# MisEty/RTG-SLAM

Hardware: AMD Instinct MI355X
Metric: hot_path_units_per_sec (higher is better)
Workload: dtype f32; 1 GPU; `value` counts UNITS, not SLAM frames (the SLAM frame rate by the reference's definition is `slam_frames_per_sec`, from the `slam_sequence` leg of --full).  One UNIT per step = 1 ICP track (3 levels x 5 GN iters, 1200x680, on a second HIP stream) + 1 map-optimisation iteration (raster fwd + masked L1 colour / gated depth loss + attach regulariser + raster bwd + fused Adam) over 1200000 random Gaus; gaussians=1200000, mode=single, parallelism=1 GPU

## Files before the change

include/rtgs_debug.h:

```cpp
#ifndef RTGS_DEBUG_H
#define RTGS_DEBUG_H
#include "rtgs_raster.h"
#ifdef __cplusplus
extern "C" {
#endif

void rtgs_raster_set_counters(void* counters);
void rtgs_raster_set_counters_ctx(rtgs_ctx* ctx, void* counters);

void rtgs_raster_set_profiling(int enable);
void rtgs_raster_set_profiling_ctx(rtgs_ctx* ctx, int enable);

void rtgs_raster_set_near_slice(int mode, int budget_per_tile);
void rtgs_raster_set_near_slice_ctx(rtgs_ctx* ctx, int mode, int budget_per_tile);

void rtgs_raster_force_sort_path(int enable);
void rtgs_raster_force_sort_path_ctx(rtgs_ctx* ctx, int enable);
int rtgs_raster_last_timings(float* ms12_host);
int rtgs_raster_last_timings_ctx(rtgs_ctx* ctx, float* ms12_host);

void rtgs_raster_set_bwd_walk_ctx(rtgs_ctx* ctx, int mode);
void rtgs_raster_set_onepass_ctx(rtgs_ctx* ctx, int on);
void rtgs_raster_set_fused_sort_ctx(rtgs_ctx* ctx, int on);
int rtgs_raster_fused_sort_stats_ctx(rtgs_ctx* ctx, int64_t* out18);
void rtgs_raster_set_tile_gather_ctx(rtgs_ctx* ctx, int mode);
int rtgs_raster_tile_gather_stats_ctx(rtgs_ctx* ctx, int64_t* out6);
void rtgs_raster_set_bwd_debug(int bits);
void rtgs_raster_set_bwd_stamps(void* dev);
void rtgs_raster_set_fwd_stamps(void* dev);
#define RTGS_ICP_STAMP_LAUNCHES 16
#define RTGS_ICP_STAMP_WGS 256
void rtgs_icp_set_stamps(void* dev);
void rtgs_tsdf_set_dense(int on);

#ifdef __cplusplus
}
#endif
#endif
```

rtg_slam_amd/csrc/map_fused.hip:

```cpp
#include "../../include/rtgs_raster.h"
#include "raster_common.h"
#include "raster_chain.h"
#include "adam_common.h"
#include "activate_common.h"

#include <math.h>

namespace rtgs {

struct FusedArgs {
  RasterParams p;
  const float *opac, *scales, *rots, *normal_w;
  const uint8_t* clamped;
  const BwdInfo* info;
  const uint32_t* gbase;
  uint32_t* slot_count;
  uint8_t* touched;
  SplatGrad* records;
  float *xyz, *shs, *raw8;
  float *m_xyz, *v_xyz, *m_shs, *v_shs, *m_raw8, *v_raw8;
  const float *lr_xyz, *lr_shs, *lr_raw8;
  uint8_t *ever_xyz, *ever_shs, *ever_raw8;
  float beta1, beta2, eps, bc1, bc2_sqrt;
  const float* init_xyz;
  const float4* init_raw8;
  const float* attach_info;
  float* confidence;
  float *act_opacity, *act_scales, *act_normal;
  float4* act_rots;
  uint32_t* live_counts;
  uint8_t* marks;
  int t0, rows;
};

constexpr int BIG_RUN = 8;

__device__ __forceinline__ bool attach_sel(const float4 init_lo) {
  return 1.f / (1.f + __expf(-init_lo.x)) < 0.9f;
}

template <int FCHUNK, int RPW = 64>
__global__ void __launch_bounds__(256) map_fused_tail_kernel(FusedArgs a) {
  __shared__ uint32_t s_list[FCHUNK];
  __shared__ uint32_t s_n;
  __shared__ float s_big[4][64][16];
  __shared__ float s_sh[4][64][20];
  __shared__ int s_rows[4][64];
  if (spec_failed(a.p.spec_fail)) return;
  const int tid = threadIdx.x, lane = tid & 63, wv = tid >> 6;
  const bool use_slots = a.info->use_slots != 0;
  const float* __restrict__ slots = reinterpret_cast<const float*>(a.info->slot_grads);
  uint32_t n_grad = 0, n_step = 0;
  for (int c0 = blockIdx.x * FCHUNK; c0 < a.rows; c0 += gridDim.x * FCHUNK) {
    __syncthreads();
    if (tid == 0) s_n = 0;
    __syncthreads();
    constexpr int PASSES = FCHUNK >= 256 ? FCHUNK / 256 : 1;
    uint32_t flags = 0;
#pragma unroll
    for (int k = 0; k < PASSES; ++k) {
      const int rl = min(c0 + k * 256 + tid, a.rows - 1);
      const uint32_t f = (uint32_t)a.touched[a.t0 + rl] | (uint32_t)a.ever_raw8[rl] | (uint32_t)a.ever_xyz[rl] | (uint32_t)a.ever_shs[rl];
      flags |= (f != 0u ? 1u : 0u) << k;
    }
#pragma unroll
    for (int k = 0; k < PASSES; ++k) {
      const int rl = c0 + k * 256 + tid;
      const bool work = rl < a.rows && k * 256 + tid < FCHUNK && ((flags >> k) & 1u) != 0u;
      const unsigned long long m = __builtin_amdgcn_ballot_w64(work);
      if (m == 0ull) continue;
      uint32_t base = 0;
      if (lane == 0) base = atomicAdd(&s_n, (uint32_t)__popcll(m));
      base = (uint32_t)__builtin_amdgcn_readfirstlane((int)base);
      if (work) s_list[base + (uint32_t)__popcll(m & ((1ull << lane) - 1ull))] = (uint32_t)rl;
    }
    __syncthreads();
    const int nlive = (int)s_n;
    for (int q0 = wv * RPW; q0 < nlive; q0 += 4 * RPW) {
      const int q = q0 + lane;
      const bool have = lane < RPW && q < nlive;
      const int rl = have ? (int)s_list[q] : 0;
      const int r = a.t0 + rl;
      bool rgrad = have && a.touched[r] != 0;
      SplatGrad g{};
      uint32_t cnt = 0, b0 = 0;
      if (rgrad && use_slots) { cnt = a.slot_count[r]; b0 = a.gbase[r]; }
      if (use_slots) {
        unsigned long long bigm = __builtin_amdgcn_ballot_w64(rgrad && cnt > (uint32_t)BIG_RUN);
        while (bigm != 0ull) {
          const int src = __builtin_ctzll(bigm);
          bigm &= bigm - 1ull;
          const uint32_t n = (uint32_t)__builtin_amdgcn_readlane((int)cnt, src);
          const size_t base = (size_t)(uint32_t)__builtin_amdgcn_readlane((int)b0, src);
          if (n <= 48u) {
            const int grp = lane >> 4, c = lane & 15;
            float m0 = 0.f, m1 = 0.f;
            uint32_t s = grp;
            for (; s + 4 < n; s += 8) { m0 += slots[(base + s) * 16 + c]; m1 += slots[(base + s + 4) * 16 + c]; }
            if (s < n) m0 += slots[(base + s) * 16 + c];
            float acc = m0 + m1;
            acc += __shfl_xor(acc, 16);
            acc += __shfl_xor(acc, 32);
            if (lane < 16) s_big[wv][src][c] = acc;
          } else {
            const float4* __restrict__ s4 = reinterpret_cast<const float4*>(slots);
            const uint32_t sub = (uint32_t)lane & 3u, sg = (uint32_t)lane >> 2;
            float4 a0 = make_float4(0.f, 0.f, 0.f, 0.f), a1 = a0, a2 = a0, a3 = a0;
            uint32_t s = sg;
            for (; s + 48 < n; s += 64) {
              const float4 t0 = s4[(base + s) * 4 + sub], t1 = s4[(base + s + 16) * 4 + sub];
              const float4 t2 = s4[(base + s + 32) * 4 + sub], t3 = s4[(base + s + 48) * 4 + sub];
              a0.x += t0.x; a0.y += t0.y; a0.z += t0.z; a0.w += t0.w; a1.x += t1.x; a1.y += t1.y; a1.z += t1.z; a1.w += t1.w;
              a2.x += t2.x; a2.y += t2.y; a2.z += t2.z; a2.w += t2.w; a3.x += t3.x; a3.y += t3.y; a3.z += t3.z; a3.w += t3.w;
            }
            for (; s < n; s += 16) {
              const float4 t0 = s4[(base + s) * 4 + sub];
              a0.x += t0.x; a0.y += t0.y; a0.z += t0.z; a0.w += t0.w;
            }
            float4 acc = make_float4((a0.x + a1.x) + (a2.x + a3.x), (a0.y + a1.y) + (a2.y + a3.y), (a0.z + a1.z) + (a2.z + a3.z),
                                     (a0.w + a1.w) + (a2.w + a3.w));
#pragma unroll
            for (int off = 4; off < 64; off <<= 1) {
              acc.x += __shfl_xor(acc.x, off); acc.y += __shfl_xor(acc.y, off);
              acc.z += __shfl_xor(acc.z, off); acc.w += __shfl_xor(acc.w, off);
            }
            if (lane < 4) { s_big[wv][src][4 * sub] = acc.x; s_big[wv][src][4 * sub + 1] = acc.y; s_big[wv][src][4 * sub + 2] = acc.z; s_big[wv][src][4 * sub + 3] = acc.w; }
          }
        }
        __builtin_amdgcn_wave_barrier();
        if (rgrad) {
          float t[16];
          if (cnt > (uint32_t)BIG_RUN) {
#pragma unroll
            for (int c = 0; c < 16; ++c) t[c] = s_big[wv][lane][c];
          } else {
#pragma unroll
            for (int c = 0; c < 16; ++c) t[c] = 0.f;
            const float4* s4 = reinterpret_cast<const float4*>(slots) + (size_t)b0 * 4;
            for (uint32_t s = 0; s < cnt; ++s) {
              const float4 x0 = s4[s * 4], x1 = s4[s * 4 + 1], x2 = s4[s * 4 + 2], x3 = s4[s * 4 + 3];
              t[0] += x0.x; t[1] += x0.y; t[2] += x0.z; t[3] += x0.w; t[4] += x1.x; t[5] += x1.y; t[6] += x1.z; t[7] += x1.w;
              t[8] += x2.x; t[9] += x2.y; t[10] += x2.z; t[11] += x2.w; t[12] += x3.x;
            }
          }
          g.du = t[0]; g.dv = t[1]; g.dca = t[2]; g.dcb = t[3]; g.dcc = t[4]; g.dop = t[5]; g.dr = t[6]; g.dg = t[7];
          g.db = t[8]; g.dnx = t[9]; g.dny = t[10]; g.dnz = t[11]; g.dpd = t[12];
          a.slot_count[r] = 0u;
        }
      } else if (rgrad) {
        g = a.records[r];
        float4* z = reinterpret_cast<float4*>(a.records + r);
        z[0] = z[1] = z[2] = z[3] = make_float4(0.f, 0.f, 0.f, 0.f);
      }
      if (rgrad) {
        a.touched[r] = 0;
        rgrad = (g.du != 0.f) | (g.dv != 0.f) | (g.dca != 0.f) | (g.dcb != 0.f) | (g.dcc != 0.f) | (g.dop != 0.f) |
                (g.dr != 0.f) | (g.dg != 0.f) | (g.db != 0.f) | (g.dnx != 0.f) | (g.dny != 0.f) | (g.dnz != 0.f) | (g.dpd != 0.f);
      }
      bool need_sh = false;
      if (have) {
        const uint8_t e_raw8 = a.ever_raw8[rl], e_xyz = a.ever_xyz[rl], e_shs = a.ever_shs[rl];
        ChainOut o{};
        if (rgrad) chain_rule(a.p, r, a.xyz, a.shs, a.scales, a.rots, a.normal_w, a.clamped, g, o, nullptr);
        const float4* raw8_4 = reinterpret_cast<const float4*>(a.raw8);
        float4 at_lo = make_float4(0.f, 0.f, 0.f, 0.f), at_hi = at_lo;
        float at[3] = {0.f, 0.f, 0.f};
        bool sel = false;
        if (a.init_raw8 && (rgrad || e_raw8 != 0 || e_xyz != 0)) {
          const float4 i_lo = a.init_raw8[2 * (size_t)rl];
          sel = attach_sel(i_lo);
          if (sel) {
            const float4 i_hi = a.init_raw8[2 * (size_t)rl + 1], c_lo = raw8_4[2 * (size_t)r], c_hi = raw8_4[2 * (size_t)r + 1];
            const float n = fmaxf(a.attach_info[0], 1.f);
            const float k3 = 2000.f / (n * 3.f), k4 = 2000.f / (n * 4.f);
            at_lo = make_float4(0.f, k3 * (c_lo.y - i_lo.y), k3 * (c_lo.z - i_lo.z), k3 * (c_lo.w - i_lo.w));
            at_hi = make_float4(k4 * (c_hi.x - i_hi.x), k4 * (c_hi.y - i_hi.y), k4 * (c_hi.z - i_hi.z), k4 * (c_hi.w - i_hi.w));
#pragma unroll
            for (int c = 0; c < 3; ++c) at[c] = k3 * (a.xyz[(size_t)r * 3 + c] - a.init_xyz[(size_t)rl * 3 + c]);
          }
        }
        const bool grad = rgrad || sel;
        if (a.marks && (grad || e_raw8 != 0 || e_xyz != 0)) a.marks[r] = 1;
        if (grad || e_raw8 != 0) {
          float4 lo = make_float4(0.f, 0.f, 0.f, 0.f), hi = lo;
          if (rgrad)
            activate8_bwd_row(raw8_4[2 * (size_t)r], raw8_4[2 * (size_t)r + 1], o.dop, o.ds[0], o.ds[1], o.ds[2], o.dq, o.dn[0],
                              o.dn[1], o.dn[2], lo, hi);
          lo.y += at_lo.y; lo.z += at_lo.z; lo.w += at_lo.w;
          hi.x += at_hi.x; hi.y += at_hi.y; hi.z += at_hi.z; hi.w += at_hi.w;
          if (e_raw8 == 0) a.ever_raw8[rl] = 1;
          float4* p4 = reinterpret_cast<float4*>(a.raw8) + 2 * (size_t)r;
          float4* m4 = reinterpret_cast<float4*>(a.m_raw8) + 2 * (size_t)rl;
          float4* v4 = reinterpret_cast<float4*>(a.v_raw8) + 2 * (size_t)rl;
          const float gg[8] = {lo.x, lo.y, lo.z, lo.w, hi.x, hi.y, hi.z, hi.w};
          float4 pp[2] = {p4[0], p4[1]}, mm[2] = {m4[0], m4[1]}, vv[2] = {v4[0], v4[1]};
          float* pf = reinterpret_cast<float*>(pp); float* mf = reinterpret_cast<float*>(mm); float* vf = reinterpret_cast<float*>(vv);
#pragma unroll
          for (int c = 0; c < 8; ++c) pf[c] = adam1(pf[c], gg[c], mf[c], vf[c], a.lr_raw8[c], a.beta1, a.beta2, a.eps, a.bc1, a.bc2_sqrt);
          p4[0] = pp[0]; p4[1] = pp[1]; m4[0] = mm[0]; m4[1] = mm[1]; v4[0] = vv[0]; v4[1] = vv[1];
          if (a.act_opacity) activate8_row_store(pp[0], pp[1], r, a.act_opacity, a.act_scales, a.act_rots, a.act_normal);
        }
        if (grad || e_xyz != 0) {
          if (e_xyz == 0) a.ever_xyz[rl] = 1;
#pragma unroll
          for (int c = 0; c < 3; ++c) {
            const size_t op = (size_t)r * 3 + c, os = (size_t)rl * 3 + c;
            float mi = a.m_xyz[os], vi = a.v_xyz[os];
            a.xyz[op] = adam1(a.xyz[op], (rgrad ? o.dm[c] : 0.f) + at[c], mi, vi, a.lr_xyz[c], a.beta1, a.beta2, a.eps, a.bc1, a.bc2_sqrt);
            a.m_xyz[os] = mi; a.v_xyz[os] = vi;
          }
        }
        if (a.confidence && rgrad) {
          if (o.basis[0] * o.gc[0] != 0.f || o.basis[0] * o.gc[1] != 0.f || o.basis[0] * o.gc[2] != 0.f) a.confidence[rl] += 1.f;
        }
        need_sh = rgrad || e_shs != 0;
        if (need_sh && e_shs == 0) a.ever_shs[rl] = 1;
        n_grad += rgrad ? 1u : 0u;
        n_step += (grad || e_raw8 != 0 || e_xyz != 0 || need_sh) ? 1u : 0u;
        const unsigned long long mask = __builtin_amdgcn_ballot_w64(need_sh);
        if (need_sh) {
          const int k = __popcll(mask & ((1ull << lane) - 1ull));
          s_rows[wv][k] = rl | (rgrad ? (1 << 30) : 0);
#pragma unroll
          for (int c = 0; c < 3; ++c) s_sh[wv][k][c] = o.gc[c];
#pragma unroll
          for (int c = 0; c < 16; ++c) s_sh[wv][k][3 + c] = o.basis[c];
        }
      }
      const unsigned long long mask = __builtin_amdgcn_ballot_w64(need_sh);
      __builtin_amdgcn_wave_barrier();
      const int n = __popcll(mask);
      const int slot = lane / 12, sub = lane - slot * 12;
      for (int k0 = 0; k0 < n; k0 += 5) {
        const int k = k0 + slot;
        if (slot < 5 && k < n) {
          const int rk = s_rows[wv][k];
          const int rlk = rk & ((1 << 30) - 1);
          const size_t op = (size_t)(a.t0 + rlk) * 12 + sub, os = (size_t)rlk * 12 + sub;
          float4 gi = make_float4(0.f, 0.f, 0.f, 0.f);
          if (rk & (1 << 30)) {
            const float* sh = s_sh[wv][k];
            const int c0 = 4 * sub;
            gi.x = sh[3 + c0 / 3] * sh[c0 % 3];
            gi.y = sh[3 + (c0 + 1) / 3] * sh[(c0 + 1) % 3];
            gi.z = sh[3 + (c0 + 2) / 3] * sh[(c0 + 2) % 3];
            gi.w = sh[3 + (c0 + 3) / 3] * sh[(c0 + 3) % 3];
          }
          const float4 pi = reinterpret_cast<const float4*>(a.shs)[op];
          float4 mi = reinterpret_cast<float4*>(a.m_shs)[os], vi = reinterpret_cast<float4*>(a.v_shs)[os], po;
          po.x = adam1(pi.x, gi.x, mi.x, vi.x, a.lr_shs[4 * sub], a.beta1, a.beta2, a.eps, a.bc1, a.bc2_sqrt);
          po.y = adam1(pi.y, gi.y, mi.y, vi.y, a.lr_shs[4 * sub + 1], a.beta1, a.beta2, a.eps, a.bc1, a.bc2_sqrt);
          po.z = adam1(pi.z, gi.z, mi.z, vi.z, a.lr_shs[4 * sub + 2], a.beta1, a.beta2, a.eps, a.bc1, a.bc2_sqrt);
          po.w = adam1(pi.w, gi.w, mi.w, vi.w, a.lr_shs[4 * sub + 3], a.beta1, a.beta2, a.eps, a.bc1, a.bc2_sqrt);
          reinterpret_cast<float4*>(a.shs)[op] = po;
          reinterpret_cast<float4*>(a.m_shs)[os] = mi;
          reinterpret_cast<float4*>(a.v_shs)[os] = vi;
        }
      }
      __builtin_amdgcn_wave_barrier();
    }
  }
  if (a.live_counts) {
#pragma unroll
    for (int off = 32; off > 0; off >>= 1) { n_grad += (uint32_t)__shfl_xor((int)n_grad, off); n_step += (uint32_t)__shfl_xor((int)n_step, off); }
    if (lane == 0 && (n_grad | n_step)) { atomicAdd(&a.live_counts[0], n_grad); atomicAdd(&a.live_counts[1], n_step); }
  }
}

}

extern "C" int rtgs_map_fused_tail(const rtgs_raster_settings* settings, const rtgs_map_step_args* s, void* geom_buffer,
                                   const void* image_buffer, const uint32_t* spec_fail, uint32_t* live_counts2, void* stream) {
  return rtgs_map_fused_tail_hint(settings, s, geom_buffer, image_buffer, spec_fail, live_counts2, 0, stream);
}

extern "C" int rtgs_map_fused_tail_hint(const rtgs_raster_settings* settings, const rtgs_map_step_args* s, void* geom_buffer,
                                        const void* image_buffer, const uint32_t* spec_fail, uint32_t* live_counts2,
                                        uint32_t listed_hint, void* stream) {
  return rtgs_map_fused_tail_marked(settings, s, geom_buffer, image_buffer, spec_fail, live_counts2, listed_hint, nullptr, stream);
}

extern "C" int rtgs_map_fused_tail_marked(const rtgs_raster_settings* settings, const rtgs_map_step_args* s, void* geom_buffer,
                                          const void* image_buffer, const uint32_t* spec_fail, uint32_t* live_counts2,
                                          uint32_t listed_hint, uint8_t* marks, void* stream) {
  using namespace rtgs;
  if (!settings || !s || !geom_buffer || !image_buffer) return RTGS_E_INVALID;
  const int32_t P = s->P;
  if (P <= 0 || s->sh_coeffs != 16 || s->step < 1) return RTGS_E_INVALID;
  int32_t t0 = 0, t1 = P;
  if (s->train_begin != 0 || s->train_end != 0) { t0 = s->train_begin; t1 = s->train_end; }
  if (t0 < 0 || t1 > P || t1 < t0) return RTGS_E_INVALID;
  if (t1 == t0) return RTGS_OK;
  FusedArgs a{};
  RasterParams& p = a.p;
  p.H = settings->image_height; p.W = settings->image_width;
  p.gx = (p.W + TILE - 1) / TILE; p.gy = (p.H + TILE - 1) / TILE;
  p.P = P; p.M = 16; p.deg = settings->sh_degree;
  p.tanfovx = settings->tanfovx; p.tanfovy = settings->tanfovy;
  p.fx = (float)(p.W / (2.0 * (double)settings->tanfovx));
  p.fy = (float)(p.H / (2.0 * (double)settings->tanfovy));
  p.cx = settings->cx > 0.f ? settings->cx : 0.5f * (float)(p.W - 1);
  p.cy = settings->cy > 0.f ? settings->cy : 0.5f * (float)(p.H - 1);
  p.scale_modifier = settings->scale_modifier;
  p.opaque_thr = settings->opaque_threshold; p.depth_thr = settings->depth_threshold; p.normal_thr = settings->normal_threshold;
  p.color_sigma = settings->color_sigma; p.T_thr = settings->T_threshold;
  p.view = settings->viewmatrix; p.campos = settings->campos; p.bg = settings->bg;
  p.spec_fail = spec_fail;
  size_t off[8];
  if (rtgs_raster_backward_buffers(P, p.H, p.W, off) != RTGS_OK) return RTGS_E_INVALID;
  const char* geom = (const char*)geom_buffer;
  const char* img = (const char*)image_buffer;
  a.opac = s->opacity; a.scales = s->scales; a.rots = s->rotations; a.normal_w = s->normal;
  a.clamped = (const uint8_t*)(geom + off[0]);
  a.gbase = (const uint32_t*)(geom + off[1]);
  a.slot_count = (uint32_t*)(geom + off[2]);
  a.info = (const BwdInfo*)(img + off[3]);
  a.records = (SplatGrad*)s->grad_scratch;
  a.touched = (uint8_t*)s->grad_scratch + off[4];
  a.xyz = s->xyz; a.shs = s->shs; a.raw8 = s->raw8;
  a.m_xyz = s->m_xyz; a.v_xyz = s->v_xyz; a.m_shs = s->m_shs; a.v_shs = s->v_shs; a.m_raw8 = s->m_raw8; a.v_raw8 = s->v_raw8;
  a.lr_xyz = s->lr_xyz; a.lr_shs = s->lr_shs; a.lr_raw8 = s->lr_raw8;
  a.ever_xyz = s->ever_xyz; a.ever_shs = s->ever_shs; a.ever_raw8 = s->ever_raw8;
  a.beta1 = s->beta1; a.beta2 = s->beta2; a.eps = s->eps;
  a.bc1 = 1.f - powf(s->beta1, (float)s->step);
  a.bc2_sqrt = sqrtf(1.f - powf(s->beta2, (float)s->step));
  if (s->attach) {
    if (!s->attach->init_xyz || !s->attach->init_raw8 || !s->attach->attach_info) return RTGS_E_INVALID;
    a.init_xyz = s->attach->init_xyz; a.init_raw8 = (const float4*)s->attach->init_raw8; a.attach_info = s->attach->attach_info;
  }
  a.confidence = s->confidence;
  a.act_opacity = s->opacity; a.act_scales = s->scales; a.act_normal = s->normal; a.act_rots = (float4*)s->rotations;
  a.live_counts = live_counts2;
  a.marks = marks;
  a.t0 = t0; a.rows = t1 - t0;
  static const int forced = [] { const char* e = getenv("RTGS_FUSED_CHUNK"); return e ? atoi(e) : 0; }();
  int chunk = 1024;
  if (forced == 512 || forced == 1024 || forced == 2048) chunk = forced;
  else if (listed_hint > 0u) {
    const double per_row = (double)listed_hint / (double)(P > 0 ? P : 1);
    chunk = per_row * 2048.0 <= 64.0 ? 2048 : (per_row * 1024.0 <= 64.0 ? 1024 : 512);
  }
  if (forced == 64 || (forced == 0 && a.rows <= 65536)) chunk = 64;
  int blocks = (a.rows + chunk - 1) / chunk;
  if (blocks > 4096) blocks = 4096;
  if (chunk == 64) hipLaunchKernelGGL((map_fused_tail_kernel<64, 16>), dim3(blocks), dim3(256), 0, (hipStream_t)stream, a);
  else if (chunk == 2048) hipLaunchKernelGGL(map_fused_tail_kernel<2048>, dim3(blocks), dim3(256), 0, (hipStream_t)stream, a);
  else if (chunk == 512) hipLaunchKernelGGL(map_fused_tail_kernel<512>, dim3(blocks), dim3(256), 0, (hipStream_t)stream, a);
  else hipLaunchKernelGGL(map_fused_tail_kernel<1024>, dim3(blocks), dim3(256), 0, (hipStream_t)stream, a);
  return hipGetLastError() == hipSuccess ? RTGS_OK : RTGS_E_HIP;
}
```

rtg_slam_amd/csrc/map_step.hip:

```cpp
#include <hip/hip_runtime.h>

#include "../../include/rtgs_raster.h"

static int map_step_front(rtgs_ctx* ctx, const rtgs_map_step_args* a, int64_t* num_rendered_host, int32_t fwd_flags,
                          void* stream, bool walk_only = false) {
  if (!a || !num_rendered_host || !a->settings) return RTGS_E_INVALID;
  const int32_t P = a->P, M = a->sh_coeffs;
  if (P <= 0 || M != 16 || a->step < 1) return RTGS_E_INVALID;
  if (!a->xyz || !a->shs || !a->raw8 || !a->tile_mask || !a->gt_color || !a->gt_depth) return RTGS_E_INVALID;
  const int32_t H = a->settings->image_height, W = a->settings->image_width;
  int rc = 0;
  if (!a->activated_valid) {
    rc = rtgs_map_activate8_forward(a->raw8, P, a->opacity, a->scales, a->rotations, a->normal, stream);
    if (rc != 0) return RTGS_E_HIP;
  }
  if (!a->loss_scratch || !a->loss4) return RTGS_E_INVALID;
  rtgs_raster_set_aux_zero_ctx(ctx, a->loss_scratch);
  rc = rtgs_raster_forward_ctx(ctx, a->settings, P, M, a->xyz, a->opacity, a->shs, a->scales, a->rotations, a->normal,
                           a->tile_mask, a->out_color, a->out_depth, a->out_color_index, a->out_depth_index,
                           a->out_color_weight, a->out_depth_weight, a->out_T, a->out_radii, a->geom_resize,
                           a->geom_user, a->binning_resize, a->binning_user, a->image_resize, a->image_user,
                           num_rendered_host, fwd_flags, stream);
  if (rc != RTGS_OK) return rc;
  void* bufs[3];
  if (rtgs_raster_last_buffers_ctx(ctx, bufs) != RTGS_OK) return RTGS_E_ALLOC;
  void *geom = bufs[0], *bin = bufs[1], *img = bufs[2];
  rtgs_loss_cfg lcfg = a->loss;
  lcfg.sums_zeroed = P > 0 ? 1 : 0;
  const bool ssim_off = a->loss.render_mask != nullptr || a->loss.ssim_weight == 0.f;
  const bool signs = walk_only && ssim_off && rtgs_raster_signs_ok_ctx(ctx, geom) != 0;
  rtgs_raster_note_loss_path_ctx(ctx, signs ? 1 : 0);
  if (signs)
    rc = rtgs_slam_loss_sums_signs(a->out_color, a->out_depth, a->out_depth_index, a->gt_color, a->gt_depth, H, W, &lcfg,
                                   a->loss_scratch, nullptr, stream);
  else
    rc = rtgs_slam_loss(a->out_color, a->out_depth, a->out_depth_index, a->gt_color, a->gt_depth, H, W, &lcfg,
                        a->loss_scratch, a->loss4, a->dL_dcolor, a->dL_ddepth, stream);
  if (rc != 0) return RTGS_E_HIP;
  int32_t t0 = 0, t1 = P;
  if (a->train_begin != 0 || a->train_end != 0) { t0 = a->train_begin; t1 = a->train_end; }
  if (t0 < 0 || t1 > P || t1 < t0) return RTGS_E_INVALID;
  if (t1 == t0)
    return signs && rtgs_slam_loss_values(&lcfg, a->loss_scratch, a->loss4, stream) != 0 ? RTGS_E_HIP : RTGS_OK;
  if (signs) {
    const rtgs_loss_signs ls{reinterpret_cast<const uint8_t*>(a->loss_scratch) + rtgs_slam_loss_signs_offset(H, W, a->loss.render_mask == nullptr),
                             reinterpret_cast<const float*>(a->loss_scratch), a->loss.color_weight, a->loss.depth_weight, a->loss4};
    return rtgs_raster_backward_walk_signs_ctx(ctx, a->settings, P, M, *num_rendered_host, a->xyz, a->opacity, a->shs, a->scales,
                                               a->rotations, a->normal, geom, bin, img, a->out_color, a->out_T, a->out_depth_index,
                                               &ls, a->grad_scratch, a->row_state, t0, t1, stream);
  }
  rc = (walk_only ? rtgs_raster_backward_walk_ctx : rtgs_raster_backward_range_ctx)(
      ctx, a->settings, P, M, *num_rendered_host, a->xyz, a->opacity, a->shs, a->scales, a->rotations, a->normal, geom, bin, img,
      a->out_color, a->out_T, a->out_depth_index, a->dL_dcolor, a->dL_ddepth, a->d_xyz, a->d_opacity, a->d_shs, a->d_scales,
      a->d_rotations, a->d_normal, a->grad_scratch, a->row_state, t0, t1, stream);
  if (rc != RTGS_OK) return rc;
  if (a->normal_weight > 0.f && a->gt_normal) {
    rc = rtgs_slam_normal_loss_range(a->normal, a->out_depth_index, a->gt_normal, a->loss.render_mask, H, W, a->normal_weight,
                                     reinterpret_cast<float*>(a->loss_scratch) + 5, a->loss4, a->d_normal, a->row_state,
                                     rtgs_raster_spec_fail_ptr_ctx(ctx), t0, t1, stream);
    if (rc != 0) return RTGS_E_HIP;
  }
  return RTGS_OK;
}

extern "C" int rtgs_slam_map_step_front_ctx(rtgs_ctx* ctx, const rtgs_map_step_args* a, int64_t* num_rendered_host,
                                            void* stream) {
  return map_step_front(ctx, a, num_rendered_host, 0, stream);
}

extern "C" int rtgs_slam_map_step_front(const rtgs_map_step_args* a, int64_t* num_rendered_host, void* stream) {
  return rtgs_slam_map_step_front_ctx(nullptr, a, num_rendered_host, stream);
}

static int map_step_once(rtgs_ctx* ctx, const rtgs_map_step_args* a, int64_t* num_rendered_host, bool speculate, void* stream) {
  const bool fused = a->tail_mode == 0 && !(a->normal_weight > 0.f && a->gt_normal);
  rtgs_raster_set_map_epoch_ctx(ctx, speculate ? a->map_epoch : 0u);
  int rc = map_step_front(ctx, a, num_rendered_host, speculate ? RTGS_FWD_SPECULATE : 0, stream, fused);
  if (rc != RTGS_OK) return rc;
  if ((a->train_begin != 0 || a->train_end != 0) && a->train_end == a->train_begin) return RTGS_OK;
  if (fused) {
    void* bufs[3];
    if (rtgs_raster_last_buffers_ctx(ctx, bufs) != RTGS_OK) return RTGS_E_ALLOC;
    return rtgs_map_fused_tail_marked(a->settings, a, bufs[0], bufs[2], rtgs_raster_spec_fail_ptr_ctx(ctx), a->live_counts,
                                      rtgs_raster_last_listed_ctx(ctx), rtgs_raster_cull_marks_ctx(ctx), stream);
  }
  const int32_t P = a->P;
  int32_t t0 = 0, t1 = P;
  if (a->train_begin != 0 || a->train_end != 0) { t0 = a->train_begin; t1 = a->train_end; }
  const size_t o = (size_t)t0;
  const rtgs_activated act{a->opacity + o, a->scales + 3 * o, a->rotations + 4 * o, a->normal + 3 * o};
  uint8_t* const marks = rtgs_raster_cull_marks_ctx(ctx);
  rc = rtgs_map_tail_rows_marked(a->xyz + 3 * o, a->shs + 48 * o, a->raw8 + 8 * o, a->d_opacity + o, a->d_scales + 3 * o,
                          a->d_rotations + 4 * o, a->d_normal + 3 * o, a->d_xyz + 3 * o, a->d_shs + 48 * o, a->d_raw8 + 8 * o,
                          a->row_state + o, a->m_xyz, a->v_xyz, a->m_shs, a->v_shs, a->m_raw8, a->v_raw8,
                          a->lr_xyz, a->lr_shs, a->lr_raw8, a->ever_xyz, a->ever_shs, a->ever_raw8, (int64_t)(t1 - t0), a->step,
                          a->beta1, a->beta2, a->eps, a->attach, a->confidence, rtgs_raster_spec_fail_ptr_ctx(ctx), &act,
                          marks ? marks + o : nullptr, stream);
  return rc != 0 ? RTGS_E_HIP : RTGS_OK;
}

extern "C" int rtgs_slam_map_step_ctx(rtgs_ctx* ctx, const rtgs_map_step_args* a, int64_t* num_rendered_host, void* stream) {
  int rc = map_step_once(ctx, a, num_rendered_host, true, stream);
  const int v = rtgs_raster_forward_verify_ctx(ctx, num_rendered_host);
  if (rc != RTGS_OK) return rc;
  if (v < 0) return v;
  if (v == 1) rc = map_step_once(ctx, a, num_rendered_host, false, stream);
  return rc;
}

extern "C" int rtgs_slam_map_step(const rtgs_map_step_args* a, int64_t* num_rendered_host, void* stream) {
  return rtgs_slam_map_step_ctx(nullptr, a, num_rendered_host, stream);
}

extern "C" size_t rtgs_map_step_args_size(void) { return sizeof(rtgs_map_step_args); }
extern "C" size_t rtgs_raster_settings_size(void) { return sizeof(rtgs_raster_settings); }

extern "C" void* rtgs_stream_create_reserving(int32_t reserve_cus) {
  int dev = 0, cus = 0;
  if (hipGetDevice(&dev) != hipSuccess) return nullptr;
  if (hipDeviceGetAttribute(&cus, hipDeviceAttributeMultiprocessorCount, dev) != hipSuccess) return nullptr;
  if (reserve_cus <= 0 || reserve_cus >= cus || cus > 1024) return nullptr;
  uint32_t mask[32] = {0};
  const int words = (cus + 31) / 32;
  for (int i = 0; i < cus - reserve_cus; ++i) mask[i >> 5] |= 1u << (i & 31);
  hipStream_t s = nullptr;
  if (hipExtStreamCreateWithCUMask(&s, (uint32_t)words, mask) != hipSuccess) return nullptr;
  return (void*)s;
}
extern "C" void rtgs_stream_destroy(void* stream) {
  if (stream) (void)hipStreamDestroy((hipStream_t)stream);
}
```

Baseline: 3093 units/s.

## Rework fused tail chunking with occupancy-aware chunk choice and packed flag scan

The fused map tail kernel now reads the four per-row flag bytes as 32-bit words, four rows per thread, and compacts live rows with multi-bit ballots. Chunk size is chosen from a wider set (up to 4096) using measured occupancy times the CUs visible to the stream. Adaptive rows-per-wave spreading and block-level aggregation of the live-count atomics are added. This is meant to cut flag-scan memory traffic and global atomics and to size the grid to the hardware. It adds a larger shared list, host-side occupancy and CU-mask queries with a mutex-guarded cache, and optional timing stamps.

```diff
diff --git a/include/rtgs_debug.h b/include/rtgs_debug.h
--- a/include/rtgs_debug.h
+++ b/include/rtgs_debug.h
@@ -28,6 +28,9 @@
 void rtgs_raster_set_bwd_debug(int bits);
 void rtgs_raster_set_bwd_stamps(void* dev);
 void rtgs_raster_set_fwd_stamps(void* dev);
+void rtgs_raster_set_tail_stamps(void* dev);
+void rtgs_raster_set_tail_shape(int chunk, int spread, int max_blocks);
+int32_t rtgs_map_fused_tail_chunk(int32_t rows, int32_t P, uint32_t listed_hint, const int32_t* slots5, int32_t* spread_out);
 #define RTGS_ICP_STAMP_LAUNCHES 16
 #define RTGS_ICP_STAMP_WGS 256
 void rtgs_icp_set_stamps(void* dev);
diff --git a/rtg_slam_amd/csrc/map_fused.hip b/rtg_slam_amd/csrc/map_fused.hip
--- a/rtg_slam_amd/csrc/map_fused.hip
+++ b/rtg_slam_amd/csrc/map_fused.hip
@@ -5,6 +5,11 @@
 #include "activate_common.h"
 
 #include <math.h>
+#include <array>
+#include <iterator>
+#include <map>
+#include <mutex>
+#include <utility>
 
 namespace rtgs {
 
@@ -31,6 +36,8 @@
   uint32_t* live_counts;
   uint8_t* marks;
   int t0, rows;
+  int shape;
+  unsigned long long* stamps;
 };
 
 constexpr int BIG_RUN = 8;
@@ -39,46 +46,78 @@
   return 1.f / (1.f + __expf(-init_lo.x)) < 0.9f;
 }
 
-template <int FCHUNK, int RPW = 64>
-__global__ void __launch_bounds__(256) map_fused_tail_kernel(FusedArgs a) {
+template <int FCHUNK, int RPW = 64, bool STAMP = false>
+__global__ void __launch_bounds__(256, (FCHUNK > 2048 || STAMP) ? 2 : 1) map_fused_tail_kernel(FusedArgs a) {
   __shared__ uint32_t s_list[FCHUNK];
   __shared__ uint32_t s_n;
   __shared__ float s_big[4][64][16];
   __shared__ float s_sh[4][64][20];
   __shared__ int s_rows[4][64];
+  __shared__ uint32_t s_cnt[2];
   if (spec_failed(a.p.spec_fail)) return;
   const int tid = threadIdx.x, lane = tid & 63, wv = tid >> 6;
   const bool use_slots = a.info->use_slots != 0;
   const float* __restrict__ slots = reinterpret_cast<const float*>(a.info->slot_grads);
   uint32_t n_grad = 0, n_step = 0;
+  if (tid == 0) s_cnt[0] = s_cnt[1] = 0u;
+  unsigned long long st_wall = 0;
+  uint32_t st_t = 0, st_list = 0, st_sum = 0, st_rest = 0;
+  uint32_t st_live = 0;
+  if constexpr (STAMP) { st_wall = wall_clock64(); st_t = (uint32_t)__builtin_readcyclecounter(); }
+#define RTGS_TAIL_LAP(INTO)                                                                                                  \
+  if constexpr (STAMP) {                                                                                                    \
+    asm volatile("s_waitcnt vmcnt(0) lgkmcnt(0)");                                                                          \
+    const uint32_t t_now = (uint32_t)__builtin_readcyclecounter();                                                          \
+    INTO += t_now - st_t; st_t = t_now;                                                                                     \
+  }
   for (int c0 = blockIdx.x * FCHUNK; c0 < a.rows; c0 += gridDim.x * FCHUNK) {
     __syncthreads();
     if (tid == 0) s_n = 0;
     __syncthreads();
-    constexpr int PASSES = FCHUNK >= 256 ? FCHUNK / 256 : 1;
+    constexpr int PASSES = FCHUNK >= 1024 ? FCHUNK / 1024 : 1;
     uint32_t flags = 0;
+    if ((a.shape & 2) != 0 && c0 + FCHUNK <= a.rows) {
+#pragma unroll
+      for (int k = 0; k < PASSES; ++k) {
+        const int i4 = (k * 256 + tid) * 4, r4 = c0 + min(i4, FCHUNK - 4);
+        const uint32_t w = *reinterpret_cast<const uint32_t*>(a.touched + a.t0 + r4) | *reinterpret_cast<const uint32_t*>(a.ever_raw8 + r4) |
+                           *reinterpret_cast<const uint32_t*>(a.ever_xyz + r4) | *reinterpret_cast<const uint32_t*>(a.ever_shs + r4);
+        const uint32_t nib = ((w & 0xffu) != 0u ? 1u : 0u) | ((w & 0xff00u) != 0u ? 2u : 0u) | ((w & 0xff0000u) != 0u ? 4u : 0u) |
+                             ((w & 0xff000000u) != 0u ? 8u : 0u);
+        flags |= (i4 < FCHUNK ? nib : 0u) << (4 * k);
+      }
+    } else {
+#pragma unroll
+      for (int k = 0; k < 4 * PASSES; ++k) {
+        const int i = ((k >> 2) * 256 + tid) * 4 + (k & 3), rl = min(c0 + i, a.rows - 1);
+        const uint32_t f = (uint32_t)a.touched[a.t0 + rl] | (uint32_t)a.ever_raw8[rl] | (uint32_t)a.ever_xyz[rl] | (uint32_t)a.ever_shs[rl];
+        flags |= (i < FCHUNK && c0 + i < a.rows && f != 0u ? 1u : 0u) << k;
+      }
+    }
 #pragma unroll
     for (int k = 0; k < PASSES; ++k) {
-      const int rl = min(c0 + k * 256 + tid, a.rows - 1);
-      const uint32_t f = (uint32_t)a.touched[a.t0 + rl] | (uint32_t)a.ever_raw8[rl] | (uint32_t)a.ever_xyz[rl] | (uint32_t)a.ever_shs[rl];
-      flags |= (f != 0u ? 1u : 0u) << k;
-    }
-#pragma unroll
-    for (int k = 0; k < PASSES; ++k) {
-      const int rl = c0 + k * 256 + tid;
-      const bool work = rl < a.rows && k * 256 + tid < FCHUNK && ((flags >> k) & 1u) != 0u;
-      const unsigned long long m = __builtin_amdgcn_ballot_w64(work);
-      if (m == 0ull) continue;
+      const uint32_t nib = (flags >> (4 * k)) & 15u, cnt = (uint32_t)__popc(nib);
+      const unsigned long long m0 = __builtin_amdgcn_ballot_w64((cnt & 1u) != 0u), m1 = __builtin_amdgcn_ballot_w64((cnt & 2u) != 0u),
+                               m2 = __builtin_amdgcn_ballot_w64((cnt & 4u) != 0u);
+      if ((m0 | m1 | m2) == 0ull) continue;
       uint32_t base = 0;
-      if (lane == 0) base = atomicAdd(&s_n, (uint32_t)__popcll(m));
+      if (lane == 0) base = atomicAdd(&s_n, (uint32_t)(__popcll(m0) + 2 * __popcll(m1) + 4 * __popcll(m2)));
       base = (uint32_t)__builtin_amdgcn_readfirstlane((int)base);
-      if (work) s_list[base + (uint32_t)__popcll(m & ((1ull << lane) - 1ull))] = (uint32_t)rl;
+      const unsigned long long below = (1ull << lane) - 1ull;
+      uint32_t pos = base + (uint32_t)(__popcll(m0 & below) + 2 * __popcll(m1 & below) + 4 * __popcll(m2 & below));
+      const int r4 = c0 + (k * 256 + tid) * 4;
+#pragma unroll
+      for (int j = 0; j < 4; ++j)
+        if ((nib >> j) & 1u) s_list[pos++] = (uint32_t)(r4 + j);
     }
     __syncthreads();
     const int nlive = (int)s_n;
-    for (int q0 = wv * RPW; q0 < nlive; q0 += 4 * RPW) {
+    const int rpw = (a.shape & 1) != 0 ? min(RPW, max(1, (nlive + 3) >> 2)) : RPW;
+    if constexpr (STAMP) st_live += (uint32_t)nlive;
+    RTGS_TAIL_LAP(st_list)
+    for (int q0 = wv * rpw; q0 < nlive; q0 += 4 * rpw) {
       const int q = q0 + lane;
-      const bool have = lane < RPW && q < nlive;
+      const bool have = lane < rpw && q < nlive;
       const int rl = have ? (int)s_list[q] : 0;
       const int r = a.t0 + rl;
       bool rgrad = have && a.touched[r] != 0;
@@ -157,6 +196,7 @@
         rgrad = (g.du != 0.f) | (g.dv != 0.f) | (g.dca != 0.f) | (g.dcb != 0.f) | (g.dcc != 0.f) | (g.dop != 0.f) |
                 (g.dr != 0.f) | (g.dg != 0.f) | (g.db != 0.f) | (g.dnx != 0.f) | (g.dny != 0.f) | (g.dnz != 0.f) | (g.dpd != 0.f);
       }
+      RTGS_TAIL_LAP(st_sum)
       bool need_sh = false;
       if (have) {
         const uint8_t e_raw8 = a.ever_raw8[rl], e_xyz = a.ever_xyz[rl], e_shs = a.ever_shs[rl];
@@ -258,14 +298,92 @@
         }
       }
       __builtin_amdgcn_wave_barrier();
+      RTGS_TAIL_LAP(st_rest)
     }
   }
   if (a.live_counts) {
 #pragma unroll
     for (int off = 32; off > 0; off >>= 1) { n_grad += (uint32_t)__shfl_xor((int)n_grad, off); n_step += (uint32_t)__shfl_xor((int)n_step, off); }
-    if (lane == 0 && (n_grad | n_step)) { atomicAdd(&a.live_counts[0], n_grad); atomicAdd(&a.live_counts[1], n_step); }
-  }
-}
+    if ((a.shape & 1) != 0) {
+      if (lane == 0 && (n_grad | n_step)) { atomicAdd(&s_cnt[0], n_grad); atomicAdd(&s_cnt[1], n_step); }
+      __syncthreads();
+      if (tid == 0 && (s_cnt[0] | s_cnt[1])) { atomicAdd(&a.live_counts[0], s_cnt[0]); atomicAdd(&a.live_counts[1], s_cnt[1]); }
+    } else if (lane == 0 && (n_grad | n_step)) {
+      atomicAdd(&a.live_counts[0], n_grad); atomicAdd(&a.live_counts[1], n_step);
+    }
+  }
+  if constexpr (STAMP) {
+    if (lane == 0) {
+      unsigned long long* o = a.stamps + (size_t)(blockIdx.x * 4 + wv) * 8;
+      o[0] = st_wall; o[1] = wall_clock64(); o[2] = st_list; o[3] = st_sum; o[4] = st_rest; o[5] = st_live; o[6] = 0; o[7] = 0;
+    }
+  }
+}
+#undef RTGS_TAIL_LAP
+
+constexpr int FUSED_CHUNKS = 5;
+static const int kFusedChunk[FUSED_CHUNKS] = {512, 1024, 2048, 3072, 4096};
+
+static int fused_chunk(int rows, int P, uint32_t listed, const int* slots, int* spread) {
+  *spread = 1;
+  if (rows <= 65536) return 64;
+  *spread = 0;
+  if (listed == 0u) return 1024;
+  const double per_row = (double)listed / (double)(P > 0 ? P : 1);
+  int chunk = kFusedChunk[0];
+  for (int i = 0; i < FUSED_CHUNKS; ++i) {
+    if (i > 0 && per_row * (double)kFusedChunk[i] > 64.0) break;
+    chunk = kFusedChunk[i];
+    if ((rows + chunk - 1) / chunk <= slots[i]) break;
+  }
+  *spread = per_row * (double)chunk <= 64.0;
+  return chunk;
+}
+
+static int tail_occupancy(int i) {
+  static const std::array<int, FUSED_CHUNKS> occ = [] {
+    std::array<int, FUSED_CHUNKS> o{};
+    const void* fn[FUSED_CHUNKS] = {(const void*)map_fused_tail_kernel<512, 64, false>, (const void*)map_fused_tail_kernel<1024, 64, false>,
+                                    (const void*)map_fused_tail_kernel<2048, 64, false>, (const void*)map_fused_tail_kernel<3072, 64, false>,
+                                    (const void*)map_fused_tail_kernel<4096, 64, false>};
+    for (int k = 0; k < FUSED_CHUNKS; ++k) {
+      int n = 0;
+      if (hipOccupancyMaxActiveBlocksPerMultiprocessor(&n, fn[k], 256, 0) != hipSuccess) { (void)hipGetLastError(); n = 0; }
+      o[k] = n;
+    }
+    return o;
+  }();
+  return occ[i];
+}
+
+static std::mutex g_cus_mu;
+static std::map<std::pair<int, void*>, int> g_cus;
+static int stream_cus(hipStream_t st) {
+  int dev = 0;
+  if (hipGetDevice(&dev) != hipSuccess) { (void)hipGetLastError(); return 0; }
+  std::lock_guard<std::mutex> lock(g_cus_mu);
+  const auto key = std::make_pair(dev, (void*)st);
+  const auto it = g_cus.find(key);
+  if (it != g_cus.end()) return it->second;
+  int cus = 0, n = 0;
+  if (hipDeviceGetAttribute(&cus, hipDeviceAttributeMultiprocessorCount, dev) != hipSuccess) { (void)hipGetLastError(); cus = 0; }
+  uint32_t mask[32] = {0};
+  if (cus > 0 && cus <= 1024 && hipExtStreamGetCUMask(st, 32, mask) == hipSuccess) {
+    for (int w = 0; w < 32; ++w) n += __builtin_popcount(mask[w]);
+  } else {
+    (void)hipGetLastError();
+  }
+  if (n <= 0 || n > cus) n = cus;
+  g_cus[key] = n;
+  return n;
+}
+void tail_forget_stream(void* stream) {
+  std::lock_guard<std::mutex> lock(g_cus_mu);
+  for (auto it = g_cus.begin(); it != g_cus.end();) it = it->first.second == stream ? g_cus.erase(it) : std::next(it);
+}
+
+static int g_tail_chunk = 0, g_tail_spread = -1, g_tail_max_blocks = 0;
+static unsigned long long* g_tail_stamps = nullptr;
 
 }
 
@@ -333,19 +451,58 @@
   a.live_counts = live_counts2;
   a.marks = marks;
   a.t0 = t0; a.rows = t1 - t0;
-  static const int forced = [] { const char* e = getenv("RTGS_FUSED_CHUNK"); return e ? atoi(e) : 0; }();
-  int chunk = 1024;
-  if (forced == 512 || forced == 1024 || forced == 2048) chunk = forced;
-  else if (listed_hint > 0u) {
-    const double per_row = (double)listed_hint / (double)(P > 0 ? P : 1);
-    chunk = per_row * 2048.0 <= 64.0 ? 2048 : (per_row * 1024.0 <= 64.0 ? 1024 : 512);
-  }
-  if (forced == 64 || (forced == 0 && a.rows <= 65536)) chunk = 64;
+  const bool words = ((reinterpret_cast<uintptr_t>(a.touched + t0) | reinterpret_cast<uintptr_t>(a.ever_raw8) | reinterpret_cast<uintptr_t>(a.ever_xyz) |
+                       reinterpret_cast<uintptr_t>(a.ever_shs)) & 3u) == 0u;
+  a.stamps = g_tail_stamps;
+  static const int env_chunk = [] { const char* e = getenv("RTGS_FUSED_CHUNK"); return e ? atoi(e) : 0; }();
+  static const int env_spread = [] { const char* e = getenv("RTGS_FUSED_SPREAD"); return e ? (atoi(e) != 0 ? 1 : 0) : -1; }();
+  if (g_tail_chunk < 0) return RTGS_OK;
+  const int forced = g_tail_chunk != 0 ? g_tail_chunk : env_chunk;
+  int spread = g_tail_spread >= 0 ? g_tail_spread : env_spread, planned_spread = 0;
+  int chunk = 0;
+  if (forced == 64) chunk = 64;
+  for (int i = 0; i < FUSED_CHUNKS; ++i)
+    if (forced == kFusedChunk[i]) chunk = forced;
+  if (chunk == 0) {
+    int slots[FUSED_CHUNKS];
+    const int cus = stream_cus((hipStream_t)stream);
+    for (int i = 0; i < FUSED_CHUNKS; ++i) slots[i] = tail_occupancy(i) * cus;
+    chunk = fused_chunk(a.rows, P, listed_hint, slots, &planned_spread);
+  } else {
+    planned_spread = chunk == 64 || (listed_hint > 0u && (double)listed_hint / (double)P * (double)chunk <= 64.0);
+  }
+  if (spread < 0) spread = planned_spread;
+  a.shape = (spread != 0 ? 1 : 0) | (words ? 2 : 0);
   int blocks = (a.rows + chunk - 1) / chunk;
   if (blocks > 4096) blocks = 4096;
-  if (chunk == 64) hipLaunchKernelGGL((map_fused_tail_kernel<64, 16>), dim3(blocks), dim3(256), 0, (hipStream_t)stream, a);
-  else if (chunk == 2048) hipLaunchKernelGGL(map_fused_tail_kernel<2048>, dim3(blocks), dim3(256), 0, (hipStream_t)stream, a);
-  else if (chunk == 512) hipLaunchKernelGGL(map_fused_tail_kernel<512>, dim3(blocks), dim3(256), 0, (hipStream_t)stream, a);
-  else hipLaunchKernelGGL(map_fused_tail_kernel<1024>, dim3(blocks), dim3(256), 0, (hipStream_t)stream, a);
+  if (g_tail_max_blocks > 0 && blocks > g_tail_max_blocks) blocks = g_tail_max_blocks;
+#define RTGS_TAIL_LAUNCH(C, R)                                                                                              \
+  do {                                                                                                                      \
+    if (a.stamps) hipLaunchKernelGGL((map_fused_tail_kernel<C, R, true>), dim3(blocks), dim3(256), 0, (hipStream_t)stream, a); \
+    else hipLaunchKernelGGL((map_fused_tail_kernel<C, R, false>), dim3(blocks), dim3(256), 0, (hipStream_t)stream, a);       \
+  } while (0)
+  switch (chunk) {
+    case 64: RTGS_TAIL_LAUNCH(64, 16); break;
+    case 512: RTGS_TAIL_LAUNCH(512, 64); break;
+    case 1024: RTGS_TAIL_LAUNCH(1024, 64); break;
+    case 2048: RTGS_TAIL_LAUNCH(2048, 64); break;
+    case 3072: RTGS_TAIL_LAUNCH(3072, 64); break;
+    default: RTGS_TAIL_LAUNCH(4096, 64); break;
+  }
+#undef RTGS_TAIL_LAUNCH
   return hipGetLastError() == hipSuccess ? RTGS_OK : RTGS_E_HIP;
 }
+
+extern "C" int32_t rtgs_map_fused_tail_chunk(int32_t rows, int32_t P, uint32_t listed_hint, const int32_t* slots5, int32_t* spread_out) {
+  if (rows <= 0 || P <= 0 || !slots5) return RTGS_E_INVALID;
+  int spread = 0;
+  const int chunk = rtgs::fused_chunk(rows, P, listed_hint, slots5, &spread);
+  if (spread_out) *spread_out = spread;
+  return chunk;
+}
+
+extern "C" void rtgs_raster_set_tail_shape(int chunk, int spread, int max_blocks) {
+  rtgs::g_tail_chunk = chunk; rtgs::g_tail_spread = spread; rtgs::g_tail_max_blocks = max_blocks;
+}
+
+extern "C" void rtgs_raster_set_tail_stamps(void* dev) { rtgs::g_tail_stamps = (unsigned long long*)dev; }
diff --git a/rtg_slam_amd/csrc/map_step.hip b/rtg_slam_amd/csrc/map_step.hip
--- a/rtg_slam_amd/csrc/map_step.hip
+++ b/rtg_slam_amd/csrc/map_step.hip
@@ -127,6 +127,8 @@
   if (hipExtStreamCreateWithCUMask(&s, (uint32_t)words, mask) != hipSuccess) return nullptr;
   return (void*)s;
 }
+namespace rtgs { void tail_forget_stream(void* stream); }
 extern "C" void rtgs_stream_destroy(void* stream) {
+  if (stream) rtgs::tail_forget_stream(stream);
   if (stream) (void)hipStreamDestroy((hipStream_t)stream);
 }
```

Result: no change. 3075 units/s (-0.6%).
